# pierotofy/OpenSplat

Hardware: NVIDIA H100
Metric: fwd_bwd_mpixel_per_s (higher is better)
Workload: dtype f32

## Files before the change

opensplat_b200/csrc/bucket.cu:

```cuda
#include "raster_common.cuh"

namespace {

constexpr int CUR_STRIDE = 32;
constexpr int BIN_THREADS = 256;
constexpr int TSCAN_THREADS = 1024;

constexpr int LEN_BUCKETS = 64;
struct BinHeader {
    unsigned ticket_n;
    unsigned ticket_t;
    unsigned done_t;
    int max_len;
    int total;
    int visible;
    int pad0[2];
    int len_hist[LEN_BUCKETS];
    int len_cur[LEN_BUCKETS];
    int pad[120];
};
static_assert(sizeof(BinHeader) == 1024, "header is 1 KB");

__device__ __forceinline__ int len_bucket(int v, int len_capacity) {
    const long long b = (long long)v * LEN_BUCKETS / ((long long)max(len_capacity, 1) + 1);
    return (int)(b < LEN_BUCKETS - 1 ? b : LEN_BUCKETS - 1);
}

constexpr unsigned long long ST_AGG = 1ull << 62, ST_INC = 2ull << 62, ST_VAL = 0xffffffffull;

__device__ __forceinline__ unsigned long long ld_state(const unsigned long long *p) {
    unsigned long long v;
    asm volatile("ld.relaxed.gpu.global.u64 %0, [%1];" : "=l"(v) : "l"(p) : "memory");
    return v;
}
__device__ __forceinline__ void st_state(unsigned long long *p, unsigned long long v) {
    asm volatile("st.relaxed.gpu.global.u64 [%0], %1;" :: "l"(p), "l"(v) : "memory");
}

__device__ __forceinline__ int chained_scan_prefix(unsigned long long *state, int blk, int aggregate) {
    const int lane = threadIdx.x & 31;
    if (blk == 0) {
        if (lane == 0) st_state(&state[0], ST_INC | (unsigned)aggregate);
        return 0;
    }
    if (lane == 0) st_state(&state[blk], ST_AGG | (unsigned)aggregate);
    int excl = 0;
    int j = blk - 1;
    while (true) {
        const int idx = j - lane;
        unsigned long long s = ST_INC;
        if (idx >= 0) s = ld_state(&state[idx]);
        const unsigned flag = (unsigned)(s >> 62);
        if (__ballot_sync(0xffffffffu, flag == 0u)) continue;
        const unsigned incm = __ballot_sync(0xffffffffu, flag == 2u);
        int val = (int)(unsigned)(s & ST_VAL);
        if (incm) {
            const int first = __ffs(incm) - 1;
            if (lane > first) val = 0;
            excl += __reduce_add_sync(0xffffffffu, val);
            break;
        }
        excl += __reduce_add_sync(0xffffffffu, val);
        j -= 32;
    }
    if (lane == 0) st_state(&state[blk], ST_INC | (unsigned)(excl + aggregate));
    return excl;
}

__global__ void __launch_bounds__(BIN_THREADS)
// ... 38 lines not shown
    __shared__ int s_blk, s_prefix;
    if (threadIdx.x == 0) s_blk = (int)atomicAdd(ticket, 1u);
    __syncthreads();
    const int blk = s_blk;
    const int e0 = (blk * BIN_THREADS + threadIdx.x) * GS_IPT;
    int v[GS_IPT];
    const bool vec = (e0 + GS_IPT <= n) && ((reinterpret_cast<uintptr_t>(counts_then_cum + e0) & 15) == 0);
    if (vec) {
        const int4 a = *reinterpret_cast<const int4 *>(counts_then_cum + e0);
        const int4 b = *reinterpret_cast<const int4 *>(counts_then_cum + e0 + 4);
        v[0] = a.x; v[1] = a.y; v[2] = a.z; v[3] = a.w; v[4] = b.x; v[5] = b.y; v[6] = b.z; v[7] = b.w;
    } else {
#pragma unroll
        for (int k = 0; k < GS_IPT; ++k) v[k] = (e0 + k < n) ? counts_then_cum[e0 + k] : 0;
    }
    int tsum = 0;
#pragma unroll
    for (int k = 0; k < GS_IPT; ++k) tsum += v[k];
    int total;
    int run = block_excl_scan<BIN_THREADS>(tsum, &total, sm);
    if (threadIdx.x < 32) {
        const int p = chained_scan_prefix(state, blk, total);
        if (threadIdx.x == 0) s_prefix = p;
    }
    __syncthreads();
    run += s_prefix;
#pragma unroll
    for (int k = 0; k < GS_IPT; ++k) { run += v[k]; v[k] = run; }
    if (vec) {
        *reinterpret_cast<int4 *>(counts_then_cum + e0) = make_int4(v[0], v[1], v[2], v[3]);
        *reinterpret_cast<int4 *>(counts_then_cum + e0 + 4) = make_int4(v[4], v[5], v[6], v[7]);
    } else {
#pragma unroll
        for (int k = 0; k < GS_IPT; ++k)
            if (e0 + k < n) counts_then_cum[e0 + k] = v[k];
    }
}

}

int gsb_count_scan_blocks(int n) { return gsb_div_up(n > 0 ? n : 1, BIN_THREADS * GS_IPT); }

void gsb_count_scan(int n, int *counts_then_cum, unsigned *ticket, unsigned long long *state, cudaStream_t s) {
    count_scan_kernel<<<gsb_count_scan_blocks(n), BIN_THREADS, 0, s>>>(n, counts_then_cum, ticket, state);
}

namespace {

__global__ void __launch_bounds__(TSCAN_THREADS)
tile_scan_kernel(int T, int nblk, int m_capacity, int len_capacity, BinHeader *hdr, unsigned long long *state,
                 int *__restrict__ tile_count_then_cursor, int2 *__restrict__ tile_bins, int *__restrict__ stats) {
    __shared__ int sm[TSCAN_THREADS / 32 + 1];
    __shared__ int s_blk, s_prefix, s_max;
    if (threadIdx.x == 0) { s_blk = (int)atomicAdd(&hdr->ticket_t, 1u); s_max = 0; }
    __syncthreads();
    const int blk = s_blk;
    const int t = blk * TSCAN_THREADS + threadIdx.x;
    const int v = (t < T) ? tile_count_then_cursor[(size_t)t * CUR_STRIDE] : 0;
    if (t < T) atomicAdd(&hdr->len_hist[len_bucket(v, len_capacity)], 1);
    int total;
    const int excl = block_excl_scan<TSCAN_THREADS>(v, &total, sm);
    const int wmax = __reduce_max_sync(0xffffffffu, v);
    if ((threadIdx.x & 31) == 0 && wmax > 0) atomicMax(&s_max, wmax);
    if (threadIdx.x < 32) {
        const int p = chained_scan_prefix(state, blk, total);
        if (threadIdx.x == 0) s_prefix = p;
    }
    __syncthreads();
    if (t < T) {
        const int e = s_prefix + excl;
        tile_bins[t] = (v > 0) ? make_int2(e, e + v) : make_int2(0, 0);
        tile_count_then_cursor[(size_t)t * CUR_STRIDE] = e;
    }
    if (threadIdx.x == 0) {
        if (s_max > 0) atomicMax(&hdr->max_len, s_max);
        if (blk == nblk - 1) atomicExch(&hdr->total, s_prefix + total);
        __threadfence();
        const unsigned done = atomicAdd(&hdr->done_t, 1u);
        if (done == (unsigned)nblk - 1u) {
            __threadfence();
            const int M = atomicAdd(&hdr->total, 0), mx = atomicAdd(&hdr->max_len, 0);
            stats[0] = M;
            stats[1] = mx;
            stats[2] = (M > m_capacity || mx > len_capacity) ? 1 : 0;
            stats[3] = hdr->visible;
        }
    }
}

__global__ void __launch_bounds__(TSCAN_THREADS)
tile_order_kernel(int T, int len_capacity, BinHeader *hdr, const int2 *__restrict__ tile_bins,
                  int *__restrict__ tile_order) {
    __shared__ int base[LEN_BUCKETS];
    if (threadIdx.x < LEN_BUCKETS) {
        int sfx = 0;
        for (int b = LEN_BUCKETS - 1; b > (int)threadIdx.x; --b) sfx += hdr->len_hist[b];
        base[threadIdx.x] = sfx;
    }
    __syncthreads();
    const int t = blockIdx.x * TSCAN_THREADS + threadIdx.x;
    if (t >= T) return;
    const int2 r = tile_bins[t];
    const int b = len_bucket(r.y - r.x, len_capacity);
    tile_order[base[b] + atomicAdd(&hdr->len_cur[b], 1)] = t;
}

__global__ void __launch_bounds__(256)
bucket_emit_kernel(int n, const GsbRecord *__restrict__ gattr, const float *__restrict__ depths,
                   const int *__restrict__ radii, const int *__restrict__ cum_tiles_hit, int cull, int tiles_x,
                   int tiles_y, int *__restrict__ cursor, unsigned long long *__restrict__ comp,
                   int *__restrict__ gaussian_ids, int *__restrict__ gid_at_pos, const int *__restrict__ stats) {
    if (stats[2]) return;
    const int i = blockIdx.x * blockDim.x + threadIdx.x;
    if (i >= n) return;
    const int r = radii[i];
    if (r <= 0) return;
    const float4 *src = reinterpret_cast<const float4 *>(gattr + i);
    const float4 q0 = src[0];
    const float hx = src[1].w, hy = src[2].w;
    int x0, x1, y0, y1;
    gsb_tile_bbox(q0.x, q0.y, (float)r, tiles_x, tiles_y, x0, x1, y0, y1);
    int k = (i == 0) ? 0 : cum_tiles_hit[i - 1];
    const unsigned long long hi = ((unsigned long long)(unsigned)__float_as_int(depths[i])) << 32;
    for (int ty = y0; ty < y1; ++ty)
        for (int tx = x0; tx < x1; ++tx) {
            if (cull && !extent_slot_mask(q0.x, q0.y, hx, hy, (float)(tx * GSB_TILE), (float)(ty * GSB_TILE)))
                continue;
            const int pos = atomicAdd(&cursor[(size_t)(ty * tiles_x + tx) * CUR_STRIDE], 1);
            comp[pos] = hi | (unsigned)k;
            if (gid_at_pos) gid_at_pos[pos] = i;
            gaussian_ids[k] = i;
            ++k;
        }
}

typedef unsigned long long u64;

constexpr int DS_MIN_BINS = 64, DS_MAX_BINS = 2048;
constexpr int DS_BIN_LIMIT = 32;

constexpr int BITONIC_MAX = 4096;

__device__ __forceinline__ u64 shfl_xor_u64(u64 v, int m) {
    unsigned lo = (unsigned)v, hi = (unsigned)(v >> 32);
    lo = __shfl_xor_sync(0xffffffffu, lo, m);
    hi = __shfl_xor_sync(0xffffffffu, hi, m);
    return ((u64)hi << 32) | lo;
}

__device__ __forceinline__ u64 cex_shfl(u64 v, int j, bool keep_min) {
    const u64 o = shfl_xor_u64(v, j);
    return ((v < o) == keep_min) ? v : o;
}

__device__ __forceinline__ void block64_substages(u64 &a, u64 &b, int base, int lane, int k, int jstart) {
    const int ia = base + lane, ib = ia + 32;
    const bool asc_a = (ia & k) == 0, asc_b = (ib & k) == 0;
    if (jstart >= 32) {
        const bool sw = (a > b) == asc_a;
        const u64 t = sw ? b : a;
        b = sw ? a : b;
        a = t;
    }
#pragma unroll
// ... 102 lines not shown
            if (k[u] >= 0) {
                q0[u].w = __int_as_float(k[u]);
                float4 *dst = reinterpret_cast<float4 *>(records + first + i);
                stg_stream4(dst, q0[u]);
                stg_stream4(dst + 1, q1[u]);
                stg_stream4(dst + 2, q2[u]);
                if (sorted_index) sorted_index[first + i] = k[u];
                if (gaussian_ids_sorted) gaussian_ids_sorted[first + i] = g[u];
            }
        }
    }
}

template <int U>
__device__ __forceinline__ void write_tile_records_g(const u64 *__restrict__ sorted, const int *__restrict__ sorted_g,
                                                     int L, int first, const GsbRecord *__restrict__ gattr,
                                                     GsbRecord *__restrict__ records, int *__restrict__ sorted_index,
                                                     int *__restrict__ gaussian_ids_sorted) {
    for (int i0 = threadIdx.x; i0 < L; i0 += U * blockDim.x) {
        float4 q0[U], q1[U], q2[U];
        int k[U], g[U];
#pragma unroll
        for (int u = 0; u < U; ++u) {
            const int i = i0 + u * blockDim.x;
            if (i < L) {
                k[u] = (int)(unsigned)(sorted[i] & 0xffffffffull);
                g[u] = sorted_g[i];
                const float4 *src = reinterpret_cast<const float4 *>(gattr + g[u]);
                q0[u] = __ldg(src); q1[u] = __ldg(src + 1); q2[u] = __ldg(src + 2);
            }
        }
#pragma unroll
        for (int u = 0; u < U; ++u) {
            const int i = i0 + u * blockDim.x;
            if (i < L) {
                q0[u].w = __int_as_float(k[u]);
                float4 *dst = reinterpret_cast<float4 *>(records + first + i);
                stg_stream4(dst, q0[u]);
                stg_stream4(dst + 1, q1[u]);
                stg_stream4(dst + 2, q2[u]);
                if (sorted_index) sorted_index[first + i] = k[u];
                if (gaussian_ids_sorted) gaussian_ids_sorted[first + i] = g[u];
            }
        }
    }
}

template <int U, bool PAYLOAD>
__global__ void __launch_bounds__(256)
tile_dsort_pack_kernel(int cap, const int2 *__restrict__ tile_bins, const unsigned long long *__restrict__ comp,
                       const int *__restrict__ gid_at_pos, const int *__restrict__ gaussian_ids,
                       const GsbRecord *__restrict__ gattr, GsbRecord *__restrict__ records,
                       int *__restrict__ sorted_index, int *__restrict__ gaussian_ids_sorted,
                       const int *__restrict__ stats, unsigned char *__restrict__ tile_done) {
    extern __shared__ unsigned long long dkey[];
    __shared__ int dhist[DS_MAX_BINS];
    __shared__ int ds_scan[256 / 32 + 1];
    __shared__ unsigned ds_lo, ds_hi;
    __shared__ int ds_maxbin;
    if (stats[2]) return;
    const int tile = blockIdx.x;
    const int2 range = tile_bins[tile];
    const int L = range.y - range.x;
    const int lane = threadIdx.x & 31;
    if (L <= 0) { if (threadIdx.x == 0) tile_done[tile] = 1; return; }
    if (L > cap) { if (threadIdx.x == 0) tile_done[tile] = 0; return; }
    u64 *in = dkey, *out = dkey + cap;
    int *gin = reinterpret_cast<int *>(dkey + 2 * cap), *gout = gin + cap;
    if (L <= 64) {
        if (threadIdx.x < 32) {
            u64 a = (lane < L) ? comp[range.x + lane] : ~0ull;
            u64 b = (32 + lane < L) ? comp[range.x + 32 + lane] : ~0ull;
#pragma unroll
            for (int k = 2; k <= 64; k <<= 1) block64_substages(a, b, 0, lane, k, k >> 1);
            out[lane] = a;
            out[32 + lane] = b;
        }
        __syncthreads();
        write_tile_records<1>(out, L, range.x, gaussian_ids, gattr, records, sorted_index, gaussian_ids_sorted);
        if (threadIdx.x == 0) tile_done[tile] = 1;
        return;
    }
    if (threadIdx.x == 0) { ds_lo = ~0u; ds_hi = 0u; ds_maxbin = 0; }
    int nb = DS_MIN_BINS;
    while (nb < (L >> 1) && nb < DS_MAX_BINS) nb <<= 1;
    for (int b = threadIdx.x; b < nb; b += blockDim.x) dhist[b] = 0;
    __syncthreads();
    unsigned lo = ~0u, hi = 0u;
    for (int i = threadIdx.x; i < L; i += blockDim.x) {
        const u64 c = comp[range.x + i];
        in[i] = c;
        if (PAYLOAD) gin[i] = gid_at_pos[range.x + i];
        const unsigned d = (unsigned)(c >> 32);
        lo = min(lo, d); hi = max(hi, d);
    }
    lo = __reduce_min_sync(0xffffffffu, lo);
    hi = __reduce_max_sync(0xffffffffu, hi);
    if (lane == 0) { atomicMin(&ds_lo, lo); atomicMax(&ds_hi, hi); }
    __syncthreads();
    if (ds_hi == ds_lo) { if (threadIdx.x == 0) tile_done[tile] = 0; return; }
    const float fmin = __uint_as_float(ds_lo);
    const float scale = (float)nb / (__uint_as_float(ds_hi) - fmin);
    auto bin_of = [&](u64 c) {
        const int b = (int)((__uint_as_float((unsigned)(c >> 32)) - fmin) * scale);
        return min(max(b, 0), nb - 1);
    };
    for (int i = threadIdx.x; i < L; i += blockDim.x) atomicAdd(&dhist[bin_of(in[i])], 1);
    __syncthreads();
    {
        int v[DS_MAX_BINS / 256], tsum = 0, tmax = 0;
#pragma unroll
        for (int q = 0; q < DS_MAX_BINS / 256; ++q) {
            const int b = threadIdx.x * (DS_MAX_BINS / 256) + q;
            v[q] = (b < nb) ? dhist[b] : 0;
            tsum += v[q]; tmax = max(tmax, v[q]);
        }
        int total;
        int run = block_excl_scan<256>(tsum, &total, ds_scan);
        tmax = __reduce_max_sync(0xffffffffu, tmax);
        if (lane == 0) atomicMax(&ds_maxbin, tmax);
#pragma unroll
        for (int q = 0; q < DS_MAX_BINS / 256; ++q) {
            const int b = threadIdx.x * (DS_MAX_BINS / 256) + q;
            if (b < nb) dhist[b] = run;
            run += v[q];
        }
    }
    __syncthreads();
    if (ds_maxbin > DS_BIN_LIMIT) { if (threadIdx.x == 0) tile_done[tile] = 0; return; }
    for (int i = threadIdx.x; i < L; i += blockDim.x) {
        const u64 c = in[i];
        const int p = atomicAdd(&dhist[bin_of(c)], 1);
        out[p] = c;
        if (PAYLOAD) gout[p] = gin[i];
    }
    __syncthreads();
    for (int b = threadIdx.x; b < nb; b += blockDim.x) {
        const int e = dhist[b], st = b ? dhist[b - 1] : 0;
        for (int p = st + 1; p < e; ++p) {
            const u64 c = out[p];
            const int cg = PAYLOAD ? gout[p] : 0;
            int q = p - 1;
            while (q >= st && out[q] > c) {
                out[q + 1] = out[q];
                if (PAYLOAD) gout[q + 1] = gout[q];
                --q;
            }
            out[q + 1] = c;
            if (PAYLOAD) gout[q + 1] = cg;
        }
    }
    __syncthreads();
    if (PAYLOAD) write_tile_records_g<U>(out, gout, L, range.x, gattr, records, sorted_index, gaussian_ids_sorted);
    else write_tile_records<U>(out, L, range.x, gaussian_ids, gattr, records, sorted_index, gaussian_ids_sorted);
    if (threadIdx.x == 0) tile_done[tile] = 1;
}

template <int MAXI>
__global__ void __launch_bounds__(256)
tile_sort_pack_kernel(int cap, const int2 *__restrict__ tile_bins, const unsigned long long *__restrict__ comp,
                      const int *__restrict__ gaussian_ids, const GsbRecord *__restrict__ gattr,
                      GsbRecord *__restrict__ records, int *__restrict__ sorted_index,
                      int *__restrict__ gaussian_ids_sorted, const int *__restrict__ stats,
                      const unsigned char *__restrict__ tile_done) {
    extern __shared__ unsigned long long skey[];
    __shared__ unsigned whist[8][256];
    __shared__ unsigned bin_base[256 + 8];
    __shared__ unsigned s_flag;
    if (stats[2]) return;
    const int tile = blockIdx.x;
    if (tile_done[tile]) return;
    const int2 range = tile_bins[tile];
    const int L = range.y - range.x;
    if (L <= 0) return;
    int n2 = 64;
    while (n2 < L) n2 <<= 1;
    if (n2 > 64 && n2 < 256) n2 = 256;
    if (n2 > cap) return;
    const int lane = threadIdx.x & 31, warp = threadIdx.x >> 5;
    for (int i = threadIdx.x; i < n2; i += blockDim.x) skey[i] = (i < L) ? comp[range.x + i] : ~0ull;
    __syncthreads();
    if (L > 1) {
        if (n2 == 64) {
            if (warp == 0) {
                u64 a = skey[lane], b = skey[32 + lane];
#pragma unroll
                for (int k = 2; k <= 64; k <<= 1) block64_substages(a, b, 0, lane, k, k >> 1);
                skey[lane] = a;
                skey[32 + lane] = b;
            }
        } else if (n2 <= BITONIC_MAX) {
            const int nwarps = blockDim.x >> 5, nblk = n2 >> 6;
            for (int blk = warp; blk < nblk; blk += nwarps) {
                const int base = blk << 6;
                u64 a = skey[base + lane], b = skey[base + 32 + lane];
#pragma unroll
                for (int k = 2; k <= 64; k <<= 1) block64_substages(a, b, base, lane, k, k >> 1);
                skey[base + lane] = a;
                skey[base + 32 + lane] = b;
            }
            __syncthreads();
            for (int k = 128; k <= n2; k <<= 1) {
                for (int j = k >> 1; j >= 64; j >>= 1) {
                    for (int t = threadIdx.x; t < (n2 >> 1); t += blockDim.x) {
                        const int lo = ((t & ~(j - 1)) << 1) | (t & (j - 1));
                        const int hiI = lo + j;
                        const bool asc = ((lo & k) == 0);
                        const u64 x = skey[lo], y = skey[hiI];
                        if ((x > y) == asc) {
                            skey[lo] = y;
                            skey[hiI] = x;
                        }
                    }
                    __syncthreads();
                }
                for (int blk = warp; blk < nblk; blk += nwarps) {
                    const int base = blk << 6;
                    u64 a = skey[base + lane], b = skey[base + 32 + lane];
                    block64_substages(a, b, base, lane, k, 32);
                    skey[base + lane] = a;
                    skey[base + 32 + lane] = b;
                }
                __syncthreads();
            }
        } else {
            const int items = n2 >> 8;
            if (items == 1) cta_radix_sort_depth<1>(skey, whist, bin_base, &s_flag);
            else if (items == 2) cta_radix_sort_depth<2>(skey, whist, bin_base, &s_flag);
            else if (items == 4) cta_radix_sort_depth<4>(skey, whist, bin_base, &s_flag);
            else if (MAXI >= 16 && items == 8) cta_radix_sort_depth<(MAXI >= 16 ? 8 : 1)>(skey, whist, bin_base, &s_flag);
            else if (MAXI >= 16 && items == 16) cta_radix_sort_depth<(MAXI >= 16 ? 16 : 1)>(skey, whist, bin_base, &s_flag);
            else if (MAXI >= 64 && items == 32) cta_radix_sort_depth<(MAXI >= 64 ? 32 : 1)>(skey, whist, bin_base, &s_flag);
            else if (MAXI >= 64) cta_radix_sort_depth<(MAXI >= 64 ? 64 : 1)>(skey, whist, bin_base, &s_flag);
            for (int i = threadIdx.x; i < L; i += blockDim.x) {
                const unsigned dep = (unsigned)(skey[i] >> 32);
                if (i > 0 && (unsigned)(skey[i - 1] >> 32) == dep) continue;
                int e = i + 1;
                while (e < L && (unsigned)(skey[e] >> 32) == dep) ++e;
                for (int p = i + 1; p < e; ++p) {
                    const u64 v = skey[p];
                    int q = p - 1;
                    while (q >= i && skey[q] > v) { skey[q + 1] = skey[q]; --q; }
                    skey[q + 1] = v;
                }
            }
        }
        __syncthreads();
    }
    write_tile_records<1>(skey, L, range.x, gaussian_ids, gattr, records, sorted_index, gaussian_ids_sorted);
}

struct BucketLayout {
    size_t hdr, state_n, state_t, cursor, zero_bytes, gattr, comp, gids, gpos, done, total;
    int nblk_n, nblk_t;
};
BucketLayout bucket_layout(int n, int m, int T) {
    BucketLayout L;
    L.nblk_n = gsb_count_scan_blocks(n);
    L.nblk_t = gsb_div_up(T > 0 ? T : 1, TSCAN_THREADS);
    size_t o = 0;
    L.hdr = o; o += sizeof(BinHeader);
    L.state_n = o; o += gsb_align_up((size_t)L.nblk_n * 8, 256);
    L.state_t = o; o += gsb_align_up((size_t)L.nblk_t * 8, 256);
    L.cursor = o; o += gsb_align_up((size_t)(T > 0 ? T : 1) * CUR_STRIDE * sizeof(int), 256);
    L.zero_bytes = o;
    L.gattr = o; o += gsb_align_up((size_t)n * sizeof(GsbRecord), 256);
    L.comp = o; o += gsb_align_up((size_t)m * 8, 256);
    L.gids = o; o += gsb_align_up((size_t)m * 4, 256);
    L.gpos = o; o += gsb_align_up((size_t)m * 4, 256);
    L.done = o; o += gsb_align_up((size_t)(T > 0 ? T : 1), 256);
    L.total = o;
    return L;
}

constexpr int BUCKET_MAX_CAP = 16384;

int sort_cap_of(int len_capacity) {
    int cap = 64;
    while (cap < len_capacity && cap < (1 << 30)) cap <<= 1;
    if (cap > 64 && cap < 256) cap = 256;
    return cap;
}

}

extern "C" int gsb_bucket_max_tile_len(void) { return BUCKET_MAX_CAP; }

extern "C" size_t gsb_bucket_workspace_bytes(int n, int m_capacity, int num_tiles) {
    return bucket_layout(n > 0 ? n : 0, m_capacity > 0 ? m_capacity : 0, num_tiles).total;
}

extern "C" int gsb_bucket_tile_ranges(int n, const float *xys, const int32_t *radii, const float *conics,
                                      const float *colors, const float *opacities, int cull, int tiles_x,
                                      int tiles_y, int m_capacity, int len_capacity, void *workspace,
                                      size_t workspace_bytes, int32_t *cum_tiles_hit, int32_t *tile_bins,
                                      int32_t *tile_order, int32_t *stats, gsb_stream_t stream) {
    GSB_CHECK_ARG(n >= 0 && tiles_x > 0 && tiles_y > 0 && m_capacity >= 0 && len_capacity >= 0);
    GSB_CHECK_ARG(tile_bins && stats && workspace && ((uintptr_t)workspace % 256) == 0);
    GSB_CHECK_ARG((cull & ~(1 | GSB_BIN_COUNT_VISIBLE)) == 0);
    const bool count_visible = (cull & GSB_BIN_COUNT_VISIBLE) != 0;
    cull &= 1;
    const int T = tiles_x * tiles_y;
    const BucketLayout L = bucket_layout(n, m_capacity, T);
    if (workspace_bytes < L.total) {
        gsb_set_error(GSB_ERR_WORKSPACE, "bucket workspace too small", __FILE__, __LINE__);
        return GSB_ERR_WORKSPACE;
    }
    cudaStream_t s = (cudaStream_t)stream;
    char *ws = (char *)workspace;
    BinHeader *hdr = (BinHeader *)(ws + L.hdr);
    int *cursor = (int *)(ws + L.cursor);
    GSB_CUDA(cudaMemsetAsync(ws, 0, L.zero_bytes, s));
    if (n > 0) {
        GSB_CHECK_ARG(xys && radii && conics && colors && opacities && cum_tiles_hit && ((uintptr_t)xys % 8) == 0);
        bin_count_kernel<<<gsb_div_up(n, BIN_THREADS), BIN_THREADS, 0, s>>>(
            n, reinterpret_cast<const float2 *>(xys), radii, conics, colors, opacities, cull, tiles_x, tiles_y, cursor,
            (GsbRecord *)(ws + L.gattr), cum_tiles_hit, count_visible ? &hdr->visible : nullptr);
        gsb_count_scan(n, cum_tiles_hit, &hdr->ticket_n, (unsigned long long *)(ws + L.state_n), s);
    }
    tile_scan_kernel<<<L.nblk_t, TSCAN_THREADS, 0, s>>>(T, L.nblk_t, m_capacity, len_capacity, hdr,
                                                       (unsigned long long *)(ws + L.state_t), cursor,
                                                       reinterpret_cast<int2 *>(tile_bins), stats);
    if (tile_order)
        tile_order_kernel<<<L.nblk_t, TSCAN_THREADS, 0, s>>>(T, len_capacity, hdr,
                                                            reinterpret_cast<const int2 *>(tile_bins), tile_order);
    GSB_LAUNCH_CHECK();
    return 0;
}

extern "C" int gsb_bucket_sort_pack(int n, int m_capacity, int len_capacity, const float *depths,
                                    const int32_t *radii, const int32_t *cum_tiles_hit, int cull, int tiles_x,
                                    int tiles_y, const int32_t *tile_bins, const int32_t *stats, void *workspace,
                                    size_t workspace_bytes, void *records, int32_t *sorted_index,
                                    int32_t *gaussian_ids_sorted, gsb_stream_t stream) {
    GSB_CHECK_ARG(n >= 0 && m_capacity >= 0 && tiles_x > 0 && tiles_y > 0 && len_capacity >= 0);
    if (n == 0 || m_capacity == 0) return 0;
    GSB_CHECK_ARG(depths && radii && cum_tiles_hit && tile_bins && stats && workspace && records);
    GSB_CHECK_ARG(((uintptr_t)workspace % 256) == 0 && ((uintptr_t)records % 16) == 0);
    const int T = tiles_x * tiles_y;
    const BucketLayout L = bucket_layout(n, m_capacity, T);
    if (workspace_bytes < L.total) {
        gsb_set_error(GSB_ERR_WORKSPACE, "bucket workspace too small", __FILE__, __LINE__);
        return GSB_ERR_WORKSPACE;
    }
    const int cap = sort_cap_of(len_capacity);
    if (cap > BUCKET_MAX_CAP) {
        gsb_set_error(GSB_ERR_UNSUPPORTED, "tile list longer than the in-shared-memory sort capacity; "
                      "use the generic gsb_sort_intersects path", __FILE__, __LINE__);
        return GSB_ERR_UNSUPPORTED;
    }
    cudaStream_t s = (cudaStream_t)stream;
    char *ws = (char *)workspace;
    unsigned long long *comp = (unsigned long long *)(ws + L.comp);
    int *gids = (int *)(ws + L.gids);
    GsbRecord *gattr = (GsbRecord *)(ws + L.gattr);
    const bool long_lists = cap > 1024;
    bucket_emit_kernel<<<gsb_div_up(n, 256), 256, 0, s>>>(n, gattr, depths, radii, cum_tiles_hit, cull, tiles_x,
                                                         tiles_y, (int *)(ws + L.cursor), comp, gids,
                                                         long_lists ? (int *)(ws + L.gpos) : nullptr, stats);
    const int dcap = cap < 8192 ? cap : 8192;
    const size_t dsmem = (size_t)dcap * (long_lists ? 24 : 16);
    unsigned char *tile_done = (unsigned char *)(ws + L.done);
#define GSB_DSP(U, PAY)                                                                                         \
    do {                                                                                                        \
        if (dsmem > 32 * 1024)                                                                                  \
            GSB_CUDA(cudaFuncSetAttribute(tile_dsort_pack_kernel<U, PAY>,                                       \
                                          cudaFuncAttributeMaxDynamicSharedMemorySize, (int)dsmem));            \
        tile_dsort_pack_kernel<U, PAY><<<T, 256, dsmem, s>>>(dcap, reinterpret_cast<const int2 *>(tile_bins), comp, \
                                                            (const int *)(ws + L.gpos), gids, gattr,            \
                                                            reinterpret_cast<GsbRecord *>(records), sorted_index, \
                                                            gaussian_ids_sorted, stats, tile_done);             \
    } while (0)
    if (long_lists) GSB_DSP(2, true);
    else GSB_DSP(1, false);
#undef GSB_DSP
    const size_t smem = (size_t)cap * 8;
#define GSB_TSP(MAXI)                                                                                           \
    do {                                                                                                        \
        if (smem > 38 * 1024)                                                                                   \
            GSB_CUDA(cudaFuncSetAttribute(tile_sort_pack_kernel<MAXI>, cudaFuncAttributeMaxDynamicSharedMemorySize, \
                                          (int)smem));                                                          \
        tile_sort_pack_kernel<MAXI><<<T, 256, smem, s>>>(                                                       \
            cap, reinterpret_cast<const int2 *>(tile_bins), comp, gids, gattr,                                  \
            reinterpret_cast<GsbRecord *>(records), sorted_index, gaussian_ids_sorted, stats, tile_done);       \
    } while (0)
    if (cap <= 1024) GSB_TSP(4);
    else if (cap <= 4096) GSB_TSP(16);
    else GSB_TSP(64);
#undef GSB_TSP
    GSB_LAUNCH_CHECK();
    return 0;
}
```

opensplat_b200/csrc/raster_bwd.cu:

```cuda
#include "raster_common.cuh"

int gsb_blend_grid(const void *kernel, int num_tiles);

namespace {

__device__ __forceinline__ float rcp_approx(float x) {
    float y;
    asm("rcp.approx.ftz.f32 %0, %1;" : "=f"(y) : "f"(x));
    return y;
}

__device__ __forceinline__ void zero_row(float *grad_rows, int k) {
    float4 *row = reinterpret_cast<float4 *>(grad_rows + (size_t)k * GSB_GRAD_ROW_FLOATS);
    const float4 z = make_float4(0.f, 0.f, 0.f, 0.f);
    row[0] = z; row[1] = z; row[2] = z;
}

constexpr int BWD_MIN_BLOCKS = 6;
constexpr int BWD_DEPTH_MIN_BLOCKS = 5;
template <bool SAT, bool DEPTH>
__global__ void __launch_bounds__(RK_THREADS, DEPTH ? BWD_DEPTH_MIN_BLOCKS : BWD_MIN_BLOCKS)
rasterize_backward_kernel(int img_h, int img_w, int tiles_x, int num_tiles,
                          const int2 *__restrict__ tile_bins, const GsbRecord *__restrict__ records,
                          const float *__restrict__ background, const float *__restrict__ final_Ts,
                          const int *__restrict__ final_idx, const float *__restrict__ v_output,
                          const float *__restrict__ v_output_alpha, float *__restrict__ grad_rows,
                          unsigned *__restrict__ tile_counter, const int *__restrict__ tile_order,
                          const float *__restrict__ record_depths, const float *__restrict__ v_output_depth) {
    __shared__ WarpRing rings[RK_WARPS];
    const int warp = threadIdx.x >> 5, lane = threadIdx.x & 31;
    WarpRing &ring = rings[warp];
    if (lane == 0) {
#pragma unroll
        for (int s = 0; s < RK_STAGES; ++s) mbar_init(&ring.full[s], 1);
        mbar_fence_init();
    }
    __syncwarp();
    const float bg0 = __ldg(background), bg1 = __ldg(background + 1), bg2 = __ldg(background + 2);
    unsigned gchunk = 0;

    while (true) {
        int tile = 0;
        if (lane == 0) tile = (int)atomicAdd(tile_counter, 1u);
        tile = __shfl_sync(0xffffffffu, tile, 0);
        if (tile >= num_tiles) break;
        if (tile_order) tile = __ldg(tile_order + tile);
        const int2 range = tile_bins[tile];
        if (range.y <= range.x) continue;

        const int tx = tile % tiles_x, ty = tile / tiles_x;
        const int X = tx * GSB_TILE + (lane & 15);
        const int Y0 = ty * GSB_TILE + (lane >> 4);
        const float px = (float)X;
        const float tile_x0 = (float)(tx * GSB_TILE), tile_y0 = (float)(ty * GSB_TILE);

        float T[RK_PIX], Bq[RK_PIX];
        const float py0 = (float)Y0;
        float vor[RK_PIX], vog[RK_PIX], vob[RK_PIX];
        float vD[RK_PIX];
        int binf[RK_PIX];
        int my_max = -1;
#pragma unroll
        for (int j = 0; j < RK_PIX; ++j) {
            const int Y = Y0 + 2 * j;
            if (X < img_w && Y < img_h) {
                const size_t p = (size_t)Y * img_w + X;
                const float Tf = final_Ts[p];
                T[j] = Tf;
                vor[j] = v_output[3 * p]; vog[j] = v_output[3 * p + 1]; vob[j] = v_output[3 * p + 2];
                binf[j] = final_idx[p];
                if (SAT) {
                    const int f = binf[j];
                    if (f & GSB_SAT_BIT0) vor[j] = 0.f;
                    if (f & (GSB_SAT_BIT0 << 1)) vog[j] = 0.f;
                    if (f & (GSB_SAT_BIT0 << 2)) vob[j] = 0.f;
                    binf[j] = f & ~GSB_SAT_MASK;
                }
                if (DEPTH) vD[j] = v_output_depth ? v_output_depth[p] : 0.f;
                const float voa = v_output_alpha ? v_output_alpha[p] : 0.f;
                Bq[j] = -(Tf * (voa - (bg0 * vor[j] + bg1 * vog[j] + bg2 * vob[j])));
            } else {
                T[j] = 1.f; vor[j] = vog[j] = vob[j] = 0.f; Bq[j] = 0.f;
                if (DEPTH) vD[j] = 0.f;
                binf[j] = -1;
            }
            my_max = max(my_max, binf[j]);
        }
        const int warp_max = __reduce_max_sync(0xffffffffu, my_max);
        const int hi = min(range.y - 1, max(warp_max, range.x - 1));

        for (int idx = hi + 1 + lane; idx < range.y; idx += 32)
            zero_row(grad_rows, __float_as_int(__ldg(&records[idx].q0.w)));
        const int L = hi - range.x + 1;
        if (L <= 0) continue;
        const int nchunks = (L + RK_CHUNK - 1) / RK_CHUNK;

        const unsigned g0 = gchunk;
        auto stage_of = [&](int c) { return (g0 + (unsigned)c) % RK_STAGES; };
        auto parity_of = [&](int c) { return ((g0 + (unsigned)c) / RK_STAGES) & 1u; };
        auto chunk_lo = [&](int c) { return max(range.x, hi + 1 - (c + 1) * RK_CHUNK); };
        auto chunk_cnt = [&](int c) { return (hi + 1 - c * RK_CHUNK) - chunk_lo(c); };
        auto issue = [&](int c) {
            if (lane == 0) {
                const unsigned s = stage_of(c);
                const uint32_t bytes = (uint32_t)chunk_cnt(c) * (uint32_t)sizeof(GsbRecord);
                mbar_arrive_expect_tx(&ring.full[s], bytes);
                tma_load_1d(&ring.rec[s][0], records + chunk_lo(c), bytes, &ring.full[s]);
            }
        };
        const int pro = min(RK_STAGES, nchunks);
        for (int c = 0; c < pro; ++c) issue(c);
        int issued = pro;

        for (int c = 0; c < nchunks; ++c) {
            const unsigned s = stage_of(c);
            float zl = 0.f;
            if (DEPTH && lane < chunk_cnt(c)) zl = __ldg(record_depths + chunk_lo(c) + lane);
            mbar_wait(&ring.full[s], parity_of(c));
            const int lo = chunk_lo(c), cnt = chunk_cnt(c);
            unsigned my_mask = 0;
            if (lane < cnt) {
                my_mask = record_slot_mask(ring.rec[s][lane], tile_x0, tile_y0);
                if (my_mask == 0u) zero_row(grad_rows, __float_as_int(ring.rec[s][lane].q0.w));
            }
            unsigned live = __ballot_sync(0xffffffffu, my_mask != 0u);
            while (live) {
                const int t = 31 - __clz(live);
                live &= ~(1u << t);
                const unsigned rm = __shfl_sync(0xffffffffu, my_mask, t);
                float z = 0.f;
                if (DEPTH) z = __shfl_sync(0xffffffffu, zl, t);
                const int idx = lo + t;
                const float4 q0 = ring.rec[s][t].q0;
                const float4 q1 = ring.rec[s][t].q1;
                const float4 q2 = ring.rec[s][t].q2;
                const float smax = fmaxf(0.f, fmaf(q0.z, GSB_LN2, GSB_SMAX_BIAS));
                const float dx = q0.x - px;
                const float adx2 = q1.x * dx * dx;
                const float bdx = q1.y * dx;
                const float dy0 = q0.y - py0;
                float s0 = 0.f, s1 = 0.f, s2 = 0.f;
                float a_r = 0.f, a_g = 0.f, a_b = 0.f;
                float a_z = 0.f;
                bool any = false;
                const int jlo = __ffs(rm) - 1, jhi = 31 - __clz(rm);
#define GSB_BWD_SLOT(j)                                                                                   \
    {                                                                                                     \
        const float dy = dy0 - (float)(2 * j);                                                                      \
        const float sigma = fmaf(dy, fmaf(q1.z, dy, bdx), adx2);                                          \
        if (__float_as_uint(sigma) <= __float_as_uint(smax)) {                    \
            const float au = ex2_approx(fmaf(sigma, -GSB_LOG2E, q0.z));           \
            const float alpha = fminf(0.99f, au);                                                         \
            if (idx <= binf[j] && alpha >= (1.f / 255.f)) {                                               \
                any = true;                                                                               \
                const float ra = rcp_approx(1.f - alpha);                                                 \
                T[j] *= ra;                                                                               \
                const float fac = alpha * T[j];                                                           \
                a_r = fmaf(fac, vor[j], a_r);                                                             \
                a_g = fmaf(fac, vog[j], a_g);                                                             \
                a_b = fmaf(fac, vob[j], a_b);                                                             \
                if (DEPTH) a_z = fmaf(fac, vD[j], a_z);                                                   \
                float d = fmaf(q2.z, vob[j], fmaf(q2.y, vog[j], q2.x * vor[j]));         \
                if (DEPTH) d = fmaf(z, vD[j], d);                                        \
                const float v_alpha = fmaf(d, T[j], -(ra * Bq[j]));                                       \
                Bq[j] = fmaf(d, fac, Bq[j]);                                                              \
                 \
                const float w = au * v_alpha;                                                             \
                const float wdy = w * dy;                                                                 \
                s0 += w;                                                                                  \
                s1 += wdy;                                                                                \
                s2 = fmaf(wdy, dy, s2);                                                                   \
            }                                                                                             \
        }                                                                                                 \
        if (jhi == j) break;                                                                              \
    }
                switch (jlo) {
                    case 0: GSB_BWD_SLOT(0)
                    case 1: GSB_BWD_SLOT(1)
                    case 2: GSB_BWD_SLOT(2)
                    case 3: GSB_BWD_SLOT(3)
                    case 4: GSB_BWD_SLOT(4)
                    case 5: GSB_BWD_SLOT(5)
                    case 6: GSB_BWD_SLOT(6)
                    default: GSB_BWD_SLOT(7)
                }
#undef GSB_BWD_SLOT
                const int k = __float_as_int(q0.w);
                float *row = grad_rows + (size_t)k * GSB_GRAD_ROW_FLOATS;
                if (!__any_sync(0xffffffffu, any)) {
                    if (lane < (DEPTH ? 10 : 9)) row[lane] = 0.f;
                    continue;
                }
                const float sx = dx * s0;
                float v0 = s0, v1 = sx, v2 = s1, v3 = dx * sx, v4 = dx * s1, v5 = s2, v6 = a_r, v7 = a_g;
                float v8 = a_b;
                {
                    const bool up = lane & 16;
                    const float t0 = up ? v0 : v4, t1 = up ? v1 : v5, t2 = up ? v2 : v6, t3 = up ? v3 : v7;
                    const float k0 = up ? v4 : v0, k1 = up ? v5 : v1, k2 = up ? v6 : v2, k3 = up ? v7 : v3;
                    v0 = k0 + __shfl_xor_sync(0xffffffffu, t0, 16);
                    v1 = k1 + __shfl_xor_sync(0xffffffffu, t1, 16);
                    v2 = k2 + __shfl_xor_sync(0xffffffffu, t2, 16);
                    v3 = k3 + __shfl_xor_sync(0xffffffffu, t3, 16);
                }
                {
                    const bool up = lane & 8;
                    const float t0 = up ? v0 : v2, t1 = up ? v1 : v3;
                    const float k0 = up ? v2 : v0, k1 = up ? v3 : v1;
                    v0 = k0 + __shfl_xor_sync(0xffffffffu, t0, 8);
                    v1 = k1 + __shfl_xor_sync(0xffffffffu, t1, 8);
                }
                {
                    const bool up = lane & 4;
                    const float t0 = up ? v0 : v1;
                    const float k0 = up ? v1 : v0;
                    v0 = k0 + __shfl_xor_sync(0xffffffffu, t0, 4);
                }
                v0 += __shfl_xor_sync(0xffffffffu, v0, 2);
                v0 += __shfl_xor_sync(0xffffffffu, v0, 1);
                if (DEPTH) {
                    const bool up = lane & 16;
                    const float t8 = up ? v8 : a_z, k8 = up ? a_z : v8;
                    v8 = k8 + __shfl_xor_sync(0xffffffffu, t8, 16);
#pragma unroll
                    for (int o = 8; o > 0; o >>= 1) v8 += __shfl_xor_sync(0xffffffffu, v8, o);
                    const bool w8 = (lane == 1), w9 = (lane == 17);
                    if (((lane & 3) == 0) || w8 || w9) row[w8 ? 8 : w9 ? 9 : (lane >> 2)] = (w8 || w9) ? v8 : v0;
                } else {
#pragma unroll
                    for (int o = 16; o > 0; o >>= 1) v8 += __shfl_xor_sync(0xffffffffu, v8, o);
                    const bool w8 = (lane == 1);
                    if (((lane & 3) == 0) || w8) row[w8 ? 8 : (lane >> 2)] = w8 ? v8 : v0;
                }
            }
            __syncwarp();
            if (issued < nchunks) { issue(issued); ++issued; }
        }
        gchunk = g0 + (unsigned)issued;
        __syncwarp();
    }
}

template <bool DEPTH>
__global__ void __launch_bounds__(256)
reduce_grad_rows_kernel(int n, const int *__restrict__ cum_tiles_hit, const float *__restrict__ grad_rows,
                        const float *__restrict__ conics, const float *__restrict__ opacities,
                        float2 *__restrict__ v_xy, float *__restrict__ v_conic,
                        float *__restrict__ v_colors, float *__restrict__ v_opacity, float *__restrict__ v_depths) {
    const int g = blockIdx.x * blockDim.x + threadIdx.x;
    if (g >= n) return;
    const int k0 = g ? cum_tiles_hit[g - 1] : 0, k1 = cum_tiles_hit[g];
    float a[9] = {0.f, 0.f, 0.f, 0.f, 0.f, 0.f, 0.f, 0.f, 0.f};
    float az = 0.f;
    for (int k = k0; k < k1; ++k) {
        const float4 *row = reinterpret_cast<const float4 *>(grad_rows + (size_t)k * GSB_GRAD_ROW_FLOATS);
        const float4 r0 = row[0], r1 = row[1];
        const float r8 = reinterpret_cast<const float *>(row)[8];
        a[0] += r0.x; a[1] += r0.y; a[2] += r0.z; a[3] += r0.w;
        a[4] += r1.x; a[5] += r1.y; a[6] += r1.z; a[7] += r1.w;
        a[8] += r8;
        if (DEPTH) az += reinterpret_cast<const float *>(row)[9];
    }
    const float S0 = a[0], Sx = a[1], Sy = a[2], Sxx = a[3], Sxy = a[4], Syy = a[5];
    const float ca = conics[3 * g], cb = conics[3 * g + 1], cc = conics[3 * g + 2];
    const float op = opacities[g];
    v_xy[g] = make_float2(-(ca * Sx + cb * Sy), -(cb * Sx + cc * Sy));
    v_conic[3 * g] = -0.5f * Sxx; v_conic[3 * g + 1] = -0.5f * Sxy; v_conic[3 * g + 2] = -0.5f * Syy;
    v_colors[3 * g] = a[6]; v_colors[3 * g + 1] = a[7]; v_colors[3 * g + 2] = a[8];
    v_opacity[g] = (op > 0.f) ? S0 / op : 0.f;
    if (DEPTH) v_depths[g] = az;
}

}

extern "C" size_t gsb_raster_grad_rows_bytes(int m) {
    return gsb_align_up((size_t)(m > 0 ? m : 0) * GSB_GRAD_ROW_FLOATS * 4 + 256, 256);
}

static int backward(int img_h, int img_w, int tiles_x, int tiles_y, int n, int m, const int32_t *tile_bins,
                    const int32_t *tile_order, const float *conics, const float *opacities, void *records,
                    const int32_t *cum_tiles_hit, const float *background, const float *final_Ts,
                    const int32_t *final_idx, const float *v_output, const float *v_output_alpha, void *grad_rows,
                    float *v_xy, float *v_conic, float *v_colors, float *v_opacity, unsigned flags, bool depth,
                    const float *record_depths, const float *v_output_depth, float *v_depths, gsb_stream_t stream) {
    GSB_CHECK_ARG(img_h > 0 && img_w > 0 && n >= 0 && m >= 0);
    GSB_CHECK_ARG((flags & ~(unsigned)GSB_RASTER_CLAMP_MAX_ONE) == 0);
    const bool sat = (flags & GSB_RASTER_CLAMP_MAX_ONE) != 0;
    GSB_CHECK_ARG(tiles_x == gsb_div_up(img_w, GSB_TILE) && tiles_y == gsb_div_up(img_h, GSB_TILE));
    if (n == 0) return 0;
    GSB_CHECK_ARG(tile_bins && conics && opacities && cum_tiles_hit && background && final_Ts && final_idx &&
// ... 58 lines not shown
```

Measured before the change: 1092.

## Compact fallback tiles into a worklist and aggregate histogram atomics in shared memory

```diff
diff --git a/opensplat_b200/csrc/bucket.cu b/opensplat_b200/csrc/bucket.cu
--- a/opensplat_b200/csrc/bucket.cu
+++ b/opensplat_b200/csrc/bucket.cu
@@ -1,3 +1,5 @@
+#include <algorithm>
+
 #include "raster_common.cuh"
 
 namespace {
@@ -14,7 +16,8 @@
     int max_len;
     int total;
     int visible;
-    int pad0[2];
+    int left_n;
+    int pad0;
     int len_hist[LEN_BUCKETS];
     int len_cur[LEN_BUCKETS];
     int pad[120];
@@ -159,12 +162,14 @@
                  int *__restrict__ tile_count_then_cursor, int2 *__restrict__ tile_bins, int *__restrict__ stats) {
     __shared__ int sm[TSCAN_THREADS / 32 + 1];
     __shared__ int s_blk, s_prefix, s_max;
+    __shared__ int s_hist[LEN_BUCKETS];
     if (threadIdx.x == 0) { s_blk = (int)atomicAdd(&hdr->ticket_t, 1u); s_max = 0; }
+    if (threadIdx.x < LEN_BUCKETS) s_hist[threadIdx.x] = 0;
     __syncthreads();
     const int blk = s_blk;
     const int t = blk * TSCAN_THREADS + threadIdx.x;
     const int v = (t < T) ? tile_count_then_cursor[(size_t)t * CUR_STRIDE] : 0;
-    if (t < T) atomicAdd(&hdr->len_hist[len_bucket(v, len_capacity)], 1);
+    if (t < T) atomicAdd(&s_hist[len_bucket(v, len_capacity)], 1);
     int total;
     const int excl = block_excl_scan<TSCAN_THREADS>(v, &total, sm);
     const int wmax = __reduce_max_sync(0xffffffffu, v);
@@ -174,6 +179,8 @@
         if (threadIdx.x == 0) s_prefix = p;
     }
     __syncthreads();
+    if (threadIdx.x < LEN_BUCKETS && s_hist[threadIdx.x] > 0)
+        atomicAdd(&hdr->len_hist[threadIdx.x], s_hist[threadIdx.x]);
     if (t < T) {
         const int e = s_prefix + excl;
         tile_bins[t] = (v > 0) ? make_int2(e, e + v) : make_int2(0, 0);
@@ -198,25 +205,35 @@
 __global__ void __launch_bounds__(TSCAN_THREADS)
 tile_order_kernel(int T, int len_capacity, BinHeader *hdr, const int2 *__restrict__ tile_bins,
                   int *__restrict__ tile_order) {
-    __shared__ int base[LEN_BUCKETS];
+    __shared__ int base[LEN_BUCKETS], cnt[LEN_BUCKETS];
     if (threadIdx.x < LEN_BUCKETS) {
         int sfx = 0;
         for (int b = LEN_BUCKETS - 1; b > (int)threadIdx.x; --b) sfx += hdr->len_hist[b];
         base[threadIdx.x] = sfx;
+        cnt[threadIdx.x] = 0;
     }
     __syncthreads();
     const int t = blockIdx.x * TSCAN_THREADS + threadIdx.x;
-    if (t >= T) return;
-    const int2 r = tile_bins[t];
-    const int b = len_bucket(r.y - r.x, len_capacity);
-    tile_order[base[b] + atomicAdd(&hdr->len_cur[b], 1)] = t;
+    int b = 0, local = 0;
+    if (t < T) {
+        const int2 r = tile_bins[t];
+        b = len_bucket(r.y - r.x, len_capacity);
+        local = atomicAdd(&cnt[b], 1);
+    }
+    __syncthreads();
+    if (threadIdx.x < LEN_BUCKETS && cnt[threadIdx.x] > 0)
+        base[threadIdx.x] += atomicAdd(&hdr->len_cur[threadIdx.x], cnt[threadIdx.x]);
+    __syncthreads();
+    if (t < T) tile_order[base[b] + local] = t;
 }
 
 __global__ void __launch_bounds__(256)
 bucket_emit_kernel(int n, const GsbRecord *__restrict__ gattr, const float *__restrict__ depths,
                    const int *__restrict__ radii, const int *__restrict__ cum_tiles_hit, int cull, int tiles_x,
                    int tiles_y, int *__restrict__ cursor, unsigned long long *__restrict__ comp,
-                   int *__restrict__ gaussian_ids, int *__restrict__ gid_at_pos, const int *__restrict__ stats) {
+                   int *__restrict__ gaussian_ids, int *__restrict__ gid_at_pos, const int *__restrict__ stats,
+                   int *__restrict__ left_n) {
+    if (blockIdx.x == 0 && threadIdx.x == 0) *left_n = 0;
     if (stats[2]) return;
     const int i = blockIdx.x * blockDim.x + threadIdx.x;
     if (i >= n) return;
@@ -425,7 +442,7 @@
                        const int *__restrict__ gid_at_pos, const int *__restrict__ gaussian_ids,
                        const GsbRecord *__restrict__ gattr, GsbRecord *__restrict__ records,
                        int *__restrict__ sorted_index, int *__restrict__ gaussian_ids_sorted,
-                       const int *__restrict__ stats, unsigned char *__restrict__ tile_done) {
+                       const int *__restrict__ stats, int *__restrict__ left_n, int *__restrict__ left) {
     extern __shared__ unsigned long long dkey[];
     __shared__ int dhist[DS_MAX_BINS];
     __shared__ int ds_scan[256 / 32 + 1];
@@ -436,8 +453,8 @@
     const int2 range = tile_bins[tile];
     const int L = range.y - range.x;
     const int lane = threadIdx.x & 31;
-    if (L <= 0) { if (threadIdx.x == 0) tile_done[tile] = 1; return; }
-    if (L > cap) { if (threadIdx.x == 0) tile_done[tile] = 0; return; }
+    if (L <= 0) return;
+    if (L > cap) { if (threadIdx.x == 0) left[atomicAdd(left_n, 1)] = tile; return; }
     u64 *in = dkey, *out = dkey + cap;
     int *gin = reinterpret_cast<int *>(dkey + 2 * cap), *gout = gin + cap;
     if (L <= 64) {
@@ -451,7 +468,6 @@
         }
         __syncthreads();
         write_tile_records<1>(out, L, range.x, gaussian_ids, gattr, records, sorted_index, gaussian_ids_sorted);
-        if (threadIdx.x == 0) tile_done[tile] = 1;
         return;
     }
     if (threadIdx.x == 0) { ds_lo = ~0u; ds_hi = 0u; ds_maxbin = 0; }
@@ -471,7 +487,7 @@
     hi = __reduce_max_sync(0xffffffffu, hi);
     if (lane == 0) { atomicMin(&ds_lo, lo); atomicMax(&ds_hi, hi); }
     __syncthreads();
-    if (ds_hi == ds_lo) { if (threadIdx.x == 0) tile_done[tile] = 0; return; }
+    if (ds_hi == ds_lo) { if (threadIdx.x == 0) left[atomicAdd(left_n, 1)] = tile; return; }
     const float fmin = __uint_as_float(ds_lo);
     const float scale = (float)nb / (__uint_as_float(ds_hi) - fmin);
     auto bin_of = [&](u64 c) {
@@ -500,7 +516,10 @@
         }
     }
     __syncthreads();
-    if (ds_maxbin > DS_BIN_LIMIT) { if (threadIdx.x == 0) tile_done[tile] = 0; return; }
+    if (ds_maxbin > DS_BIN_LIMIT) {
+        if (threadIdx.x == 0) left[atomicAdd(left_n, 1)] = tile;
+        return;
+    }
     for (int i = threadIdx.x; i < L; i += blockDim.x) {
         const u64 c = in[i];
         const int p = atomicAdd(&dhist[bin_of(c)], 1);
@@ -526,23 +545,18 @@
     __syncthreads();
     if (PAYLOAD) write_tile_records_g<U>(out, gout, L, range.x, gattr, records, sorted_index, gaussian_ids_sorted);
     else write_tile_records<U>(out, L, range.x, gaussian_ids, gattr, records, sorted_index, gaussian_ids_sorted);
-    if (threadIdx.x == 0) tile_done[tile] = 1;
 }
 
 template <int MAXI>
-__global__ void __launch_bounds__(256)
-tile_sort_pack_kernel(int cap, const int2 *__restrict__ tile_bins, const unsigned long long *__restrict__ comp,
-                      const int *__restrict__ gaussian_ids, const GsbRecord *__restrict__ gattr,
-                      GsbRecord *__restrict__ records, int *__restrict__ sorted_index,
-                      int *__restrict__ gaussian_ids_sorted, const int *__restrict__ stats,
-                      const unsigned char *__restrict__ tile_done) {
-    extern __shared__ unsigned long long skey[];
+__device__ __noinline__ void sort_pack_tile(int tile, int cap, const int2 *__restrict__ tile_bins,
+                                            const unsigned long long *__restrict__ comp,
+                                            const int *__restrict__ gaussian_ids,
+                                            const GsbRecord *__restrict__ gattr, GsbRecord *__restrict__ records,
+                                            int *__restrict__ sorted_index, int *__restrict__ gaussian_ids_sorted,
+                                            unsigned long long *skey) {
     __shared__ unsigned whist[8][256];
     __shared__ unsigned bin_base[256 + 8];
     __shared__ unsigned s_flag;
-    if (stats[2]) return;
-    const int tile = blockIdx.x;
-    if (tile_done[tile]) return;
     const int2 range = tile_bins[tile];
     const int L = range.y - range.x;
     if (L <= 0) return;
@@ -623,8 +637,25 @@
     write_tile_records<1>(skey, L, range.x, gaussian_ids, gattr, records, sorted_index, gaussian_ids_sorted);
 }
 
+template <int MAXI>
+__global__ void __launch_bounds__(256)
+tile_sort_pack_kernel(int cap, const int2 *__restrict__ tile_bins, const unsigned long long *__restrict__ comp,
+                      const int *__restrict__ gaussian_ids, const GsbRecord *__restrict__ gattr,
+                      GsbRecord *__restrict__ records, int *__restrict__ sorted_index,
+                      int *__restrict__ gaussian_ids_sorted, const int *__restrict__ stats,
+                      const int *__restrict__ left_n, const int *__restrict__ left) {
+    extern __shared__ unsigned long long skey[];
+    if (stats[2]) return;
+    const int nleft = *left_n;
+    for (int j = blockIdx.x; j < nleft; j += gridDim.x) {
+        sort_pack_tile<MAXI>(left[j], cap, tile_bins, comp, gaussian_ids, gattr, records, sorted_index,
+                             gaussian_ids_sorted, skey);
+        __syncthreads();
+    }
+}
+
 struct BucketLayout {
-    size_t hdr, state_n, state_t, cursor, zero_bytes, gattr, comp, gids, gpos, done, total;
+    size_t hdr, state_n, state_t, cursor, zero_bytes, gattr, comp, gids, gpos, left, total;
     int nblk_n, nblk_t;
 };
 BucketLayout bucket_layout(int n, int m, int T) {
@@ -641,7 +672,7 @@
     L.comp = o; o += gsb_align_up((size_t)m * 8, 256);
     L.gids = o; o += gsb_align_up((size_t)m * 4, 256);
     L.gpos = o; o += gsb_align_up((size_t)m * 4, 256);
-    L.done = o; o += gsb_align_up((size_t)(T > 0 ? T : 1), 256);
+    L.left = o; o += gsb_align_up((size_t)(T > 0 ? T : 1) * sizeof(int), 256);
     L.total = o;
     return L;
 }
@@ -728,12 +759,12 @@
     int *gids = (int *)(ws + L.gids);
     GsbRecord *gattr = (GsbRecord *)(ws + L.gattr);
     const bool long_lists = cap > 1024;
+    int *left_n = &((BinHeader *)(ws + L.hdr))->left_n, *left = (int *)(ws + L.left);
     bucket_emit_kernel<<<gsb_div_up(n, 256), 256, 0, s>>>(n, gattr, depths, radii, cum_tiles_hit, cull, tiles_x,
                                                          tiles_y, (int *)(ws + L.cursor), comp, gids,
-                                                         long_lists ? (int *)(ws + L.gpos) : nullptr, stats);
+                                                         long_lists ? (int *)(ws + L.gpos) : nullptr, stats, left_n);
     const int dcap = cap < 8192 ? cap : 8192;
     const size_t dsmem = (size_t)dcap * (long_lists ? 24 : 16);
-    unsigned char *tile_done = (unsigned char *)(ws + L.done);
 #define GSB_DSP(U, PAY)                                                                                         \
     do {                                                                                                        \
         if (dsmem > 32 * 1024)                                                                                  \
@@ -742,7 +773,7 @@
         tile_dsort_pack_kernel<U, PAY><<<T, 256, dsmem, s>>>(dcap, reinterpret_cast<const int2 *>(tile_bins), comp, \
                                                             (const int *)(ws + L.gpos), gids, gattr,            \
                                                             reinterpret_cast<GsbRecord *>(records), sorted_index, \
-                                                            gaussian_ids_sorted, stats, tile_done);             \
+                                                            gaussian_ids_sorted, stats, left_n, left);          \
     } while (0)
     if (long_lists) GSB_DSP(2, true);
     else GSB_DSP(1, false);
@@ -753,10 +784,16 @@
         if (smem > 38 * 1024)                                                                                   \
             GSB_CUDA(cudaFuncSetAttribute(tile_sort_pack_kernel<MAXI>, cudaFuncAttributeMaxDynamicSharedMemorySize, \
                                           (int)smem));                                                          \
-        tile_sort_pack_kernel<MAXI><<<T, 256, smem, s>>>(                                                       \
+        int per_sm = 1;                                                                                         \
+        GSB_CUDA(cudaOccupancyMaxActiveBlocksPerMultiprocessor(&per_sm, tile_sort_pack_kernel<MAXI>, 256, smem)); \
+        const int grid = std::max(1, std::min(T, std::max(per_sm, 1) * sms));                                   \
+        tile_sort_pack_kernel<MAXI><<<grid, 256, smem, s>>>(                                                    \
             cap, reinterpret_cast<const int2 *>(tile_bins), comp, gids, gattr,                                  \
-            reinterpret_cast<GsbRecord *>(records), sorted_index, gaussian_ids_sorted, stats, tile_done);       \
+            reinterpret_cast<GsbRecord *>(records), sorted_index, gaussian_ids_sorted, stats, left_n, left);    \
     } while (0)
+    int dev = 0, sms = 1;
+    GSB_CUDA(cudaGetDevice(&dev));
+    GSB_CUDA(cudaDeviceGetAttribute(&sms, cudaDevAttrMultiProcessorCount, dev));
     if (cap <= 1024) GSB_TSP(4);
     else if (cap <= 4096) GSB_TSP(16);
     else GSB_TSP(64);
```

New measurement: 1095 (median of 6 runs). Within noise of the previous version (+0.3%).

## Batch per-Gaussian warp reductions through shared-memory staging instead of shuffle trees

Applied to the files above, without the earlier changes.

```diff
diff --git a/opensplat_b200/csrc/raster_bwd.cu b/opensplat_b200/csrc/raster_bwd.cu
--- a/opensplat_b200/csrc/raster_bwd.cu
+++ b/opensplat_b200/csrc/raster_bwd.cu
@@ -18,6 +18,14 @@
 
 constexpr int BWD_MIN_BLOCKS = 6;
 constexpr int BWD_DEPTH_MIN_BLOCKS = 5;
+
+constexpr int BWD_BATCH = 3;
+constexpr int BWD_STAGE_ROW = 36;
+struct __align__(16) BwdStage {
+    float part[BWD_BATCH][6][BWD_STAGE_ROW];
+    int k[BWD_BATCH];
+};
+
 template <bool SAT, bool DEPTH>
 __global__ void __launch_bounds__(RK_THREADS, DEPTH ? BWD_DEPTH_MIN_BLOCKS : BWD_MIN_BLOCKS)
 rasterize_backward_kernel(int img_h, int img_w, int tiles_x, int num_tiles,
@@ -27,9 +35,28 @@
                           const float *__restrict__ v_output_alpha, float *__restrict__ grad_rows,
                           unsigned *__restrict__ tile_counter, const int *__restrict__ tile_order,
                           const float *__restrict__ record_depths, const float *__restrict__ v_output_depth) {
+    constexpr int NV = DEPTH ? 10 : 9;
     __shared__ WarpRing rings[RK_WARPS];
+    __shared__ BwdStage stages[RK_WARPS];
     const int warp = threadIdx.x >> 5, lane = threadIdx.x & 31;
     WarpRing &ring = rings[warp];
+    BwdStage &st = stages[warp];
+    int nst = 0;
+    auto flush = [&]() {
+        __syncwarp();
+        if (lane < nst * NV) {
+            const int r = lane / NV, v = lane - r * NV;
+            const float4 *src = reinterpret_cast<const float4 *>(v < 6 ? &st.part[r][v][0] : &st.part[r][v - 6][16]);
+            float sum = 0.f;
+#pragma unroll 2
+            for (int i = 0; i < 4; ++i) {
+                const float4 a = src[i];
+                sum += (a.x + a.y) + (a.z + a.w);
+            }
+            grad_rows[(size_t)st.k[r] * GSB_GRAD_ROW_FLOATS + v] = sum;
+        }
+        __syncwarp();
+    };
     if (lane == 0) {
 #pragma unroll
         for (int s = 0; s < RK_STAGES; ++s) mbar_init(&ring.full[s], 1);
@@ -51,8 +78,7 @@
         const int tx = tile % tiles_x, ty = tile / tiles_x;
         const int X = tx * GSB_TILE + (lane & 15);
         const int Y0 = ty * GSB_TILE + (lane >> 4);
-        const float px = (float)X;
-        const float tile_x0 = (float)(tx * GSB_TILE), tile_y0 = (float)(ty * GSB_TILE);
+        const float tile_x0 = (float)(tx * GSB_TILE);
 
         float T[RK_PIX], Bq[RK_PIX];
         const float py0 = (float)Y0;
@@ -120,7 +146,7 @@
             const int lo = chunk_lo(c), cnt = chunk_cnt(c);
             unsigned my_mask = 0;
             if (lane < cnt) {
-                my_mask = record_slot_mask(ring.rec[s][lane], tile_x0, tile_y0);
+                my_mask = record_slot_mask(ring.rec[s][lane], tile_x0, py0 - (float)(lane >> 4));
                 if (my_mask == 0u) zero_row(grad_rows, __float_as_int(ring.rec[s][lane].q0.w));
             }
             unsigned live = __ballot_sync(0xffffffffu, my_mask != 0u);
@@ -135,7 +161,7 @@
                 const float4 q1 = ring.rec[s][t].q1;
                 const float4 q2 = ring.rec[s][t].q2;
                 const float smax = fmaxf(0.f, fmaf(q0.z, GSB_LN2, GSB_SMAX_BIAS));
-                const float dx = q0.x - px;
+                const float dx = q0.x - (tile_x0 + (float)(lane & 15));
                 const float adx2 = q1.x * dx * dx;
                 const float bdx = q1.y * dx;
                 const float dy0 = q0.y - py0;
@@ -186,56 +212,31 @@
                 }
 #undef GSB_BWD_SLOT
                 const int k = __float_as_int(q0.w);
-                float *row = grad_rows + (size_t)k * GSB_GRAD_ROW_FLOATS;
                 if (!__any_sync(0xffffffffu, any)) {
-                    if (lane < (DEPTH ? 10 : 9)) row[lane] = 0.f;
+                    if (lane < NV) grad_rows[(size_t)k * GSB_GRAD_ROW_FLOATS + lane] = 0.f;
                     continue;
                 }
-                const float sx = dx * s0;
-                float v0 = s0, v1 = sx, v2 = s1, v3 = dx * sx, v4 = dx * s1, v5 = s2, v6 = a_r, v7 = a_g;
-                float v8 = a_b;
-                {
-                    const bool up = lane & 16;
-                    const float t0 = up ? v0 : v4, t1 = up ? v1 : v5, t2 = up ? v2 : v6, t3 = up ? v3 : v7;
-                    const float k0 = up ? v4 : v0, k1 = up ? v5 : v1, k2 = up ? v6 : v2, k3 = up ? v7 : v3;
-                    v0 = k0 + __shfl_xor_sync(0xffffffffu, t0, 16);
-                    v1 = k1 + __shfl_xor_sync(0xffffffffu, t1, 16);
-                    v2 = k2 + __shfl_xor_sync(0xffffffffu, t2, 16);
-                    v3 = k3 + __shfl_xor_sync(0xffffffffu, t3, 16);
-                }
-                {
-                    const bool up = lane & 8;
-                    const float t0 = up ? v0 : v2, t1 = up ? v1 : v3;
-                    const float k0 = up ? v2 : v0, k1 = up ? v3 : v1;
-                    v0 = k0 + __shfl_xor_sync(0xffffffffu, t0, 8);
-                    v1 = k1 + __shfl_xor_sync(0xffffffffu, t1, 8);
-                }
-                {
-                    const bool up = lane & 4;
-                    const float t0 = up ? v0 : v1;
-                    const float k0 = up ? v1 : v0;
-                    v0 = k0 + __shfl_xor_sync(0xffffffffu, t0, 4);
-                }
-                v0 += __shfl_xor_sync(0xffffffffu, v0, 2);
-                v0 += __shfl_xor_sync(0xffffffffu, v0, 1);
-                if (DEPTH) {
-                    const bool up = lane & 16;
-                    const float t8 = up ? v8 : a_z, k8 = up ? a_z : v8;
-                    v8 = k8 + __shfl_xor_sync(0xffffffffu, t8, 16);
-#pragma unroll
-                    for (int o = 8; o > 0; o >>= 1) v8 += __shfl_xor_sync(0xffffffffu, v8, o);
-                    const bool w8 = (lane == 1), w9 = (lane == 17);
-                    if (((lane & 3) == 0) || w8 || w9) row[w8 ? 8 : w9 ? 9 : (lane >> 2)] = (w8 || w9) ? v8 : v0;
-                } else {
-#pragma unroll
-                    for (int o = 16; o > 0; o >>= 1) v8 += __shfl_xor_sync(0xffffffffu, v8, o);
-                    const bool w8 = (lane == 1);
-                    if (((lane & 3) == 0) || w8) row[w8 ? 8 : (lane >> 2)] = w8 ? v8 : v0;
-                }
+                const bool up = lane & 16;
+                const float u0 = (up ? a_r : s0) + __shfl_xor_sync(0xffffffffu, up ? s0 : a_r, 16);
+                const float u1 = (up ? a_g : s1) + __shfl_xor_sync(0xffffffffu, up ? s1 : a_g, 16);
+                const float u2 = (up ? a_b : s2) + __shfl_xor_sync(0xffffffffu, up ? s2 : a_b, 16);
+                float uz = 0.f;
+                if (DEPTH) uz = a_z + __shfl_xor_sync(0xffffffffu, a_z, 16);
+                const float sx = dx * u0;
+                float *dst = &st.part[nst][0][lane];
+                dst[0] = u0;
+                dst[BWD_STAGE_ROW] = up ? u1 : sx;
+                dst[2 * BWD_STAGE_ROW] = up ? u2 : u1;
+                dst[3 * BWD_STAGE_ROW] = (DEPTH && up) ? uz : dx * sx;
+                dst[4 * BWD_STAGE_ROW] = dx * u1;
+                dst[5 * BWD_STAGE_ROW] = u2;
+                if (lane == 0) st.k[nst] = k;
+                if (++nst == BWD_BATCH) { flush(); nst = 0; }
             }
             __syncwarp();
             if (issued < nchunks) { issue(issued); ++issued; }
         }
+        if (nst) { flush(); nst = 0; }
         gchunk = g0 + (unsigned)issued;
         __syncwarp();
     }
```

Result: faster. 1091 before, 1105 after, median of 6 (+1.3%).
